# TIXhjq/ML_Function

Measured on AMD Instinct MI355X. Metric: samples/sec fwd+bwd xDeepFM-CIN B=4096,F=39,K=16, higher is better.
Workload: dtype f32

## Files before the change

ml_function_amd/csrc/cin.hip:

```cpp
#include "cin_layout.h"

namespace fil {

static const char* kFwdNames[kCinMaxL] = {"cin_fwd_l1", "cin_fwd_l2", "cin_fwd_l3", "cin_fwd_l4", "cin_fwd_l5", "cin_fwd_l6", "cin_fwd_l7", "cin_fwd_l8"};
static const char* kDwNames[kCinMaxL] = {"cin_bwd_dw_l1", "cin_bwd_dw_l2", "cin_bwd_dw_l3", "cin_bwd_dw_l4", "cin_bwd_dw_l5", "cin_bwd_dw_l6", "cin_bwd_dw_l7", "cin_bwd_dw_l8"};
static const char* kDzNames[kCinMaxL] = {"cin_bwd_dz_l1", "cin_bwd_dz_l2", "cin_bwd_dz_l3", "cin_bwd_dz_l4", "cin_bwd_dz_l5", "cin_bwd_dz_l6", "cin_bwd_dz_l7", "cin_bwd_dz_l8"};
static double gemm_flops(long M, int Hp, int F, int H) { return 2.0 * (double)M * Hp * F * H; }

static int launch_dw3(hipStream_t st, const DwPlan& p, const float* gT, int HS, const float* xT, const float* xpT, int xps, float* part,
                      long M, int F, int Hp, int H, int symD = 0, int xtra = 0) {
  const int items = p.blocks_x * p.splits * p.chunks;
  const dim3 grid((items + 7) / 8 * 8);
#define FIL_DW3(MBV, ONES) \
  hipLaunchKernelGGL((cin_dw3_kernel<MBV, ONES>), grid, dim3(kCinThreads), 0, st, gT, HS, xT, xpT, xps, part, (int)M, F, Hp, H, p.rows_per_split, \
                     p.blocks_x, p.chunks, items, symD, xtra)
  if (xT == nullptr) {
    if (p.MB == 2) FIL_DW3(2, true); else FIL_DW3(1, true);
  } else {
    if (p.MB == 2) FIL_DW3(2, false); else FIL_DW3(1, false);
  }
#undef FIL_DW3
  return p.splits;
}

// ... 461 lines not shown
struct CinBwd : CinCall {
  const float *pooled, *g;
  float* dx;
  float* const* dW;
  float* const* dbias;
  float *ddense_w, *ddense_b;
  void* const* events;
  CinBwdWs ws;
  const float* dPsrc;
  int nblk, ncol, ndc;
  int ready_slot[kCinMaxL + 1];
  int nready = 0;
  int cur = 0;
  int ltop;
  bool dx_started = false;
  bool have_gx0 = false;
  bool wz_prepacked = false;
  bool qm_joined = false;
};

static void cin_record_ready(const CinBwd& c, int slot) {
  if (c.events != nullptr && c.events[slot] != nullptr) (void)hipEventRecord((hipEvent_t)c.events[slot], c.st);
}
static void ready_next(CinBwd& c) { cin_record_ready(c, c.ready_slot[c.nready++]); }

static int cin_bwd_head(CinBwd& c) {
  const int B = c.s.B, LK = c.s.L * c.s.K;
  hipStream_t st = c.st;
  c.dPsrc = c.g;
  if (c.output_dim == 1 && c.p.qmerge) {
    c.dPsrc = c.ws.dP;
  } else if (c.output_dim == 1) {
    ProfScope ps("cin_head_bwd", st);
    hipLaunchKernelGGL(cin_head_bwd_kernel, dim3(c.nblk), dim3(256), 0, st, c.g, c.dense_w, c.pooled, c.ws.dP, c.ws.small, B, LK, kHeadChunk);
    if (!c.p.tail)
      hipLaunchKernelGGL(cin_reduce_kernel, dim3(cdiv(LK + 1, 64)), dim3(256), 0, st, c.ws.small, c.ddense_w, (long)(LK + 1), c.nblk, c.ddense_b, (long)LK);
    FIL_CIN_BWD_LAUNCHED();
    c.dPsrc = c.ws.dP;
  }
  if (!c.p.tail) ready_next(c);
  return FIL_OK;
}

static void cin_qtail_params_fill(const CinBwd& c) {
  const TailGeom& tg = c.p.tg;
  const CinBwdWs& ws = c.ws;
  const int F = c.s.F, p = tg.p, lL = c.s.L - 1, Hpp = tg.Hpp, Hq = tg.Hq;
  ProfScope ps("cin_tail_params", c.st);
  const size_t sh = cin_qtail_params_lds(F, Hq);
  allow_lds(cin_qtail_params_kernel, sh);
  float* dcfin = ws.dcpart + (size_t)c.ndc * kQtConst;
  hipLaunchKernelGGL(cin_qtail_params_kernel, dim3(2 * Hpp + 1), dim3(256), sh, c.st, c.W[p], c.sv.wsumL, ws.dT, ws.vlast, c.dW[p], ws.part, Hpp, F, Hq, ws.dcpart, c.ndc,
                     dcfin);
  hipLaunchKernelGGL(cin_qtail_fill_kernel, dim3(cdiv(Hq * F, kQtFillCols)), dim3(kQtFillThreads), 0, c.st, ws.part, Hpp, dcfin, c.bias[p], c.sv.wsumL, c.dW[lL], c.dbias[p],
                     c.dbias[lL], F, Hq, tg.HL);
}

static int cin_bwd_top_merged_q(CinBwd& c) {
  const CinShape& s = c.s;
  const TailGeom& tg = c.p.tg;
  const CinSaved& sv = c.sv;
  const CinBwdWs& ws = c.ws;
  const int F = s.F, K = s.K, L = s.L, JT = s.JT(), LK = s.L * s.K, *H = s.H;
  const long M = s.M();
  const bool qsplit = c.p.qsplit;
  const float* xT = c.xT;
  hipStream_t st = c.st;
  const int p = tg.p, lL = L - 1, Hpp = tg.Hpp, Hq = tg.Hq, HS0 = s.HS(0);
  FIL_CIN_CHECK_ARG(c.bias && c.W[0] && c.W[p] && c.W[lL] && c.bias[p] && c.dW[0] && c.dW[p] && c.dW[lL] && c.dbias[0] && c.dbias[p] && c.dbias[lL]);
  const float* xpT = sv.maps[p - 1];
  const int xps = s.xps(p);
  const float* dPp = c.dPsrc + (size_t)p * K;
  const float* dPL = c.dPsrc + (size_t)lL * K;
  const float* dPprev = c.dPsrc + (size_t)(p - 1) * K;
  const double algo_tail = gemm_flops(M, Hpp, F, Hq) + gemm_flops(M, Hq, F, tg.HL);
  const double algo1 = gemm_flops(M, F, F, H[0]);
  const int symD = F / 2 + 1, Cl = F * symD;
  const int JTs = cin_jt_sym(F);
  const int periods = cin_dz_periods(F, JTs), tiles0 = cin_slot_tiles(F, JTs);
  const bool ghat = cin_ghat_used(s, c.p, c.output_dim);
  const CinBwdWs::Scratch v = ws.scratch(s, true, ghat);
  const float* G = ghat ? sv.R : ws.G[c.cur];
  const float* gsc = ghat ? c.g : nullptr;
  {
    ProfScope ps("cin_tail_a", st, (double)M * (2 * F + 3) * sizeof(float));
    const size_t sh = (size_t)256 * (F + 3 + (c.output_dim == 1 ? L : 0) + (ghat ? 1 : 0)) * sizeof(float);
    allow_lds(cin_qtail_xe_kernel<3>, sh);
    allow_lds(cin_qtail_xe_kernel<1>, sh);
    const int np = (int)std::min<long>(((long)tiles0 * 32 * HS0 + 255) / 256, 1024);
    const int nq2 = qsplit ? 2 * std::min(cdiv(tiles0 * 512, 256), 256) : 0;
    if (c.p.qnp == 1)
      hipLaunchKernelGGL(cin_qtail_xe_kernel<1>, dim3(c.ndc + np + nq2), dim3(kXeThreads), sh, st, xT, dPL, dPp, LK, K, v.xr, ws.dcpart, (int)M, F,
                         c.ndc, c.output_dim == 1 ? c.g : nullptr, c.dense_w, c.pooled, ws.dP, ws.hpart, LK, lL, p, c.W[0], ws.Wz, H[0], JTs, HS0, tiles0, np, sv.T,
                         Hpp, ws.Wzb1, ws.Wzb2, ghat ? 1 : 0);
    else
      hipLaunchKernelGGL(cin_qtail_xe_kernel<3>, dim3(c.ndc + np + nq2), dim3(kXeThreads), sh, st, xT, dPL, dPp, LK, K, v.xr, ws.dcpart, (int)M, F,
                         c.ndc, c.output_dim == 1 ? c.g : nullptr, c.dense_w, c.pooled, ws.dP, ws.hpart, LK, lL, p, c.W[0], ws.Wz, H[0], JTs, HS0, tiles0, np, sv.T,
                         Hpp, ws.Wzb1, ws.Wzb2, ghat ? 1 : 0);
  }
  FIL_CIN_BWD_LAUNCHED();
  {
    ProfScope ps("cin_last_bwd", st, 6.0 * (double)M * Hpp * F);
    if (ghat)
      cin_launch_last_bwd2(st, JT, xT, xpT, xps, sv.wsumP, sv.wsnP, dPp, LK, nullptr, nullptr, HS0, ws.dxT, (int)M, F, K, Hpp);
    else
      cin_launch_last_bwd2(st, JT, xT, xpT, xps, sv.wsumP, sv.wsnP, dPp, LK, dPprev, ws.G[c.cur], HS0, ws.dxT, (int)M, F, K, Hpp, sv.R, HS0, dPL, ws.small);
  }
  FIL_CIN_BWD_LAUNCHED();
  int dw_parts = 0;
  {
    ProfScope ps("cin_bwd_dw_q", st, algo1 + algo_tail, gemm_flops(M, 1, Cl, H[0]) + gemm_flops(M, 1, Cl, Hpp));
    if (qsplit) {
      const DwqbPlan bp = cin_dwqb_plan(M, Cl + F, cu_count());
      cin_launch_dwq_b(st, c.p.qnp, bp, G, xpT, HS0, v.xr, v.XS, ws.part, (int)M, F, symD);
      dw_parts = bp.splits;
    } else {
      const bool f4 = knobs().dwfold4 != 0;
      const int Cw = Cl + F + (ghat ? 1 : 0);
      const DwqPlan dp = f4 ? cin_dwq_plan4(M, Cw, cu_count()) : cin_dwq_plan(M, Cw, cu_count());
#define FIL_DWQ(FOLDV, GHV) \
  hipLaunchKernelGGL((cin_dwq_kernel<kDwqDepth, FOLDV, GHV>), dim3((dp.wgs + 7) / 8 * 8), dim3(kDwqThreads), 0, st, G, xpT, HS0, v.xr, v.XS, ws.part, (int)M, F, \
                     symD, dp.rows_per_split, dp.splits, dp.ncol_full, dp.rem, dp.wgs_full, dp.wgs)
      if (ghat) {
        if (f4) FIL_DWQ(4, true); else FIL_DWQ(2, true);
      } else {
        if (f4) FIL_DWQ(4, false); else FIL_DWQ(2, false);
      }
#undef FIL_DWQ
      dw_parts = dp.pairs;
    }
  }
  FIL_CIN_BWD_LAUNCHED();
  {
    ProfScope ps("cin_reduce_dw", st);
    const int nb1 = ghat ? 0 : cdiv(H[0], 64);
    const int nh = c.output_dim == 1 ? cdiv(LK + 1, 64) : 0;
    if (ghat)
      hipLaunchKernelGGL(cin_reduce_expand_q_kernel<true>, dim3((Cl + F + 1 + 3) / 4 + nh), dim3(256), 0, st, ws.part, dw_parts, F, symD, H[0], Hpp, c.dW[0], ws.dT,
                         ws.vlast, ws.small, c.ncol, c.dbias[0], nb1, ws.hpart, c.ndc, LK, c.ddense_w, c.ddense_b);
    else
      hipLaunchKernelGGL(cin_reduce_expand_q_kernel<false>, dim3((Cl + F + 3) / 4 + nb1 + nh), dim3(256), 0, st, ws.part, dw_parts, F, symD, H[0], Hpp, c.dW[0], ws.dT,
                         ws.vlast, ws.small, c.ncol, c.dbias[0], nb1, ws.hpart, c.ndc, LK, c.ddense_w, c.ddense_b);
  }
  FIL_CIN_BWD_LAUNCHED();
  ready_next(c);
  ready_next(c);
  cin_qtail_params_fill(c);
  FIL_CIN_BWD_LAUNCHED();
  ready_next(c);
  ready_next(c);
  const int NHMAX = HS0 / 2;
  if (NHMAX == 64 && knobs().dz2 != 0) {
    ProfScope ps("cin_bwd_dz_q", st, algo1 + algo_tail, gemm_flops(M, 1, Cl, H[0]) + gemm_flops(M, 1, Cl, Hpp));
    bool split_done = false;
    if (qsplit) {
      split_done = cin_launch_dz2_b(st, c.p.qnp, JTs, G, xpT, HS0, dPL, LK, K, ws.Wzb1, ws.Wzb2, xT, ws.dxT, 1, (int)M, F, H[0], Hpp, periods, c.dx, sv.cvec);
    }
    if (!split_done &&
        !cin_launch_dz2(st, JTs, G, xpT, HS0, dPL, LK, K, ws.Wz, sv.WzT, xT, ws.dxT, 1, (int)M, F, H[0], Hpp, periods, c.dx, sv.cvec, gsc))
      return fail(FIL_ERR_UNSUPPORTED, "fil_cin_bwd: no two-pass data-gradient kernel for JT=%d (F=%d)", JTs, F);
    c.qm_joined = true;
  } else {
    const DzsShape z = dzs_launch_shape(c.p.tune, M, JTs, NHMAX);
    {
      ProfScope ps("cin_bwd_dz_tail", st, algo_tail, gemm_flops(M, 1, Cl, Hpp));
      cin_launch_dz3_sym(st, z.MBs, JTs, NHMAX, z.grid, xpT, HS0, sv.WzT, xT, v.gxR, v.dxR, 0, (int)M, F, Hpp, periods, z.ks);
    }
    FIL_CIN_BWD_LAUNCHED();
    {
      ProfScope ps("cin_bwd_dz_l1", st, algo1, gemm_flops(M, 1, Cl, H[0]));
      cin_launch_dz3_sym(st, z.MBs, JTs, NHMAX, z.grid, G, HS0, ws.Wz, xT, ws.gx0T, ws.dxT, 1, (int)M, F, H[0], periods, z.ks);
    }
    c.have_gx0 = true;
  }
  FIL_CIN_BWD_LAUNCHED();
  c.dx_started = true;
  c.ltop = -1;
  return FIL_OK;
}

static int cin_bwd_top_qtail(CinBwd& c) {
  const CinShape& s = c.s;
  const TailGeom& tg = c.p.tg;
  const CinSaved& sv = c.sv;
// ... 334 lines not shown
```

ml_function_amd/csrc/cin_layout.h:

```cpp
#pragma once
#include "cin_kernels.h"
#include "cin_tail.h"
#include "cin_launch.h"
#include "cin_qtail.h"
#include "cin_qsplit.h"
#include "cin_qmerge.h"

#include <stdlib.h>

namespace fil {

struct CinShape {
  int B, F, K, L;
  int H[kCinMaxL];
  int Hp(int l) const { return l == 0 ? F : H[l - 1]; }
  int HS(int l) const { return 128 * cdiv(H[l], 128); }
  int xps(int l) const { return l == 0 ? F : HS(l - 1); }
  long M() const { return (long)B * K; }
  int JT() const { return cin_jt_of(F); }
  int HSmax() const {
    int h = 0;
    for (int l = 0; l < L; ++l) h = std::max(h, HS(l));
    return h;
  }
};

static int check_shape(const char* fn, int B, int F, int K, int L, const int* H, CinShape& s) {
  if (B < 0 || F < 1 || K < 1 || L < 1 || H == nullptr) return fail(FIL_ERR_ARG, "%s: bad shape B=%d F=%d K=%d L=%d", fn, B, F, K, L);
  if (L > kCinMaxL) return fail(FIL_ERR_UNSUPPORTED, "%s: L=%d > %d", fn, L, kCinMaxL);
  if (F > kCinMaxFields) return fail(FIL_ERR_UNSUPPORTED, "%s: F=%d > %d fields", fn, F, kCinMaxFields);
  if ((long)B * K > (1L << 28)) return fail(FIL_ERR_UNSUPPORTED, "%s: B*K = %ld rows > 2^28 (row-split byte offsets of the dW kernel are 32-bit)", fn, (long)B * K);
  s.B = B; s.F = F; s.K = K; s.L = L;
  for (int l = 0; l < L; ++l) {
    if (H[l] < 1) return fail(FIL_ERR_ARG, "%s: H[%d]=%d", fn, l, H[l]);
    if (H[l] > kCinMaxH) return fail(FIL_ERR_UNSUPPORTED, "%s: H[%d]=%d > %d feature maps", fn, l, H[l], kCinMaxH);
    s.H[l] = H[l];
  }
  return FIL_OK;
}

static int chunks_of(int H) { return cdiv(H, 128); }
static int env_int(const char* name, int dflt) {
  const char* v = getenv(name);
  return v != nullptr && *v != 0 ? atoi(v) : dflt;
}
struct Knobs {
  int mb, sym, dw_mb, dw_splits, dz_mb, tail_splits, tail_settle, tail_dz_mode, ksplit, dzs_mb, qtail, qmerge, dz2, fwdq, headfold, packfold, dwfold4, ghat;
};
static const Knobs& knobs() {
  static const Knobs k = {env_int("FIL_CIN_MB", 0), env_int("FIL_CIN_SYM", 1), env_int("FIL_CIN_DW_MB", 1), env_int("FIL_CIN_DW_SPLITS", 0),
                          env_int("FIL_CIN_DZ_MB", 1), env_int("FIL_CIN_TAIL_SPLITS", 0), env_int("FIL_CIN_TAIL_SETTLE", 0), env_int("FIL_CIN_TAIL_DZ_MODE", 0), env_int("FIL_CIN_KSPLIT", -1), env_int("FIL_CIN_DZS_MB", 0), env_int("FIL_CIN_QTAIL", 1), env_int("FIL_CIN_QMERGE", 1), env_int("FIL_CIN_DZ2", 1), env_int("FIL_CIN_FWDQ", 1), env_int("FIL_CIN_HEADFOLD", 1), env_int("FIL_CIN_PACKFOLD", 1), env_int("FIL_CIN_DWFOLD4", 1), env_int("FIL_CIN_GHAT", 1)};
  return k;
}
struct CinTune {
  int mb_forced;
  bool sym, no_ksplit;
  CinTune() : CinTune(0) {}
  explicit CinTune(int mode)
      : mb_forced((mode & FIL_CIN_MB2) ? 2 : knobs().mb), sym(knobs().sym != 0 && !(mode & FIL_CIN_NOSYM)), no_ksplit((mode & FIL_CIN_NOKSPLIT) != 0) {}
  int mb_rows(long M) const {
    if (mb_forced == 1 || mb_forced == 2) return mb_forced;
    return cdiv((int)std::min<long>(M, 1L << 30), 64) >= 768 ? 2 : 1;
  }
  int ksplit(long M) const {
    if (knobs().ksplit == 0 || no_ksplit) return 1;
    if (mb_rows(M) != 1) return 1;
    if (knobs().ksplit == 4) return 4;
    return cdiv((int)std::min<long>(M, 1L << 30), 32) <= 512 ? 4 : 1;
  }
};

struct DwPlan {
  int MB, blocks_x, splits, rows_per_split, chunks;
};
static int cu_count() {
  static const int n = [] {
    int dev = 0, v = 0;
    if (hipGetDevice(&dev) != hipSuccess || hipDeviceGetAttribute(&v, hipDeviceAttributeMultiprocessorCount, dev) != hipSuccess || v <= 0) v = 256;
    return v;
  }();
  return n;
}

static DwPlan dw_plan(long M, int C, int H) {
  DwPlan p;
  p.chunks = chunks_of(H);
  p.MB = knobs().dw_mb == 2 ? 2 : 1;
  const int waves_c = cdiv(C, 32 * p.MB);
  p.blocks_x = cdiv(waves_c, 4);
  const long tiles = (long)p.blocks_x * p.chunks;
  const long ncu = cu_count();
  const long unit = 2 * kDwDepth;
  auto rows_of = [&](int splits) { return std::max<long>(unit, ((M + splits - 1) / splits + unit - 1) / unit * unit); };
  int best = knobs().dw_splits;
  if (best <= 0) {
    static const double t_of[4] = {0.0, 1.05e-4, 1.39e-4, 1.96e-4};
    double best_ms = -1.0;
    for (int sp = (int)std::max<long>(1, (M + (1L << 20) - 1) >> 20); sp <= 256; ++sp) {
      const long rps = rows_of(sp);
      const long real = (M + rps - 1) / rps;
      if (real != sp && sp > 1) continue;
      long wgs = tiles * real;
      double per_row = 0.0;
      while (wgs > 0) {
        const long round = std::min(wgs, 3 * ncu);
        per_row += t_of[std::min<long>(3, (round + ncu - 1) / ncu)];
        wgs -= round;
      }
      const double ms = (double)rps * per_row * p.MB + (double)real * C * H * 4.0 / 6e9;
      if (best_ms < 0 || ms < best_ms) best = sp, best_ms = ms;
      if (rps == unit) break;
    }
  }
  best = std::min(std::max(best, 1), 256);
  const long rps = rows_of(best);
  p.rows_per_split = (int)rps;
  p.splits = (int)std::max<long>(1, (M + rps - 1) / rps);
  return p;
}

struct TailGeom {
  bool on = false;
  int p = 0;
  int NCB = 0, JP = 0, JT4 = 0, NQ = 0, JHp = 0;
  int Hpp = 0, Hq = 0, HL = 0, Cp = 0, C1 = 0;
  int periods = 0, tiles = 0;
  size_t uf_floats = 0, uz_floats = 0;
};
static TailGeom tail_geom(const CinShape& s) {
  TailGeom g;
  if (s.L < 3 || !cin_tail_supported(s.F)) return g;
  g.on = true;
  g.p = s.L - 2;
  g.NCB = cin_tail_ncb(s.F);
// ... 192 lines not shown
```

ml_function_amd/csrc/cin_qmerge.h:

```cpp
#pragma once
#include "cin_kernels.h"
#include "cin_launch.h"
#include "cin_qtail.h"

namespace fil {

constexpr int kDwqDepth = 6;
constexpr int kDwqThreads = 512;
struct DwqPlan {
  int tiles, ncol_full, rem, splits, pairs, rows_per_split, wgs_full, wgs;
};
inline int cin_dwq_rem_wgs(int rem, int pairs) { return rem == 0 ? 0 : (rem == 1 ? (pairs + 3) / 4 : (rem == 2 ? (pairs + 1) / 2 : pairs)); }
inline DwqPlan cin_dwq_plan(long M, int C, int cus) {
  DwqPlan p;
  p.tiles = (C + 31) / 32;
  p.ncol_full = p.tiles / 4;
  p.rem = p.tiles % 4;
  const long unit = 2 * kDwqDepth;
  const long slots = cus;
  int best = 1;
  for (int s = 1; s <= 512; ++s) {
    if ((long)p.ncol_full * s + cin_dwq_rem_wgs(p.rem, s) > slots) break;
    best = s;
  }
// ... 191 lines not shown
  }
  float* pout = part + (long)pair * C * 256;
#pragma unroll
  for (int reg = 0; reg < 16; ++reg) {
    const int cr = c0 + mfma32_row(reg, half);
    if (cr < C) {
      float* dst = pout + (long)cr * 256 + 4 * r;
      if (cr < Cp || (GHAT && cr == C - 1)) *reinterpret_cast<float4*>(dst) = make_float4(acc[0][reg], acc[1][reg], acc[2][reg], acc[3][reg]);
      *reinterpret_cast<float4*>(dst + 128) = make_float4(acc[4][reg], acc[5][reg], acc[6][reg], acc[7][reg]);
    }
  }
}

template <bool GHAT = false>
static __global__ __launch_bounds__(256) void cin_reduce_expand_q_kernel(const float* __restrict__ part, int parts, int F, int D, int H1, int H2,
                                                                          float* __restrict__ dW1, float* __restrict__ dT, float* __restrict__ vT,
                                                                          const float* __restrict__ bpart, int nbp, float* __restrict__ dbias1,
                                                                          int nb1, const float* __restrict__ hpart, int nhp, int LK,
                                                                          float* __restrict__ ddw, float* __restrict__ ddb) {
  const int Cp = F * D, C = Cp + F + (GHAT ? 1 : 0);
  const int nbw = (C + 3) / 4;
  if ((int)blockIdx.x >= nbw + nb1) {
    cin_reduce_body(hpart, ddw, (long)LK + 1, nhp, ddb, (long)LK, (int)blockIdx.x - nbw - nb1);
    return;
  }
  if ((int)blockIdx.x >= nbw) {
    cin_reduce_body(bpart, dbias1, (long)H1, nbp, nullptr, 0, (int)blockIdx.x - nbw);
    return;
  }
  const int lane = threadIdx.x & 63, wave = threadIdx.x >> 6;
  const int c = blockIdx.x * 4 + wave;
  if (c >= C) return;
  const long ps = (long)C * 256;
  const float* p0 = part + (long)c * 256 + 4 * lane;
  f32x4 t[8];
#pragma unroll
  for (int u = 0; u < 8; ++u) t[u] = f32x4{0.f, 0.f, 0.f, 0.f};
  int p = 0;
  for (; p + 7 < parts; p += 8) {
#pragma unroll
    for (int u = 0; u < 8; ++u) t[u] += *reinterpret_cast<const f32x4*>(p0 + (long)(p + u) * ps);
  }
  for (; p < parts; ++p) t[0] += *reinterpret_cast<const f32x4*>(p0 + (long)p * ps);
  const f32x4 v = ((t[0] + t[1]) + (t[2] + t[3])) + ((t[4] + t[5]) + (t[6] + t[7]));
  const int col = 4 * lane, n0 = col & 127;
  const bool second = col >= 128;
  const int H = second ? H2 : H1;
  if (GHAT && c >= Cp + F) {
    if (!second) {
#pragma unroll
      for (int e = 0; e < 4; ++e)
        if (n0 + e < H1) dbias1[n0 + e] = v[e];
    }
    return;
  }
  if (c >= Cp) {
    if (second) {
#pragma unroll
      for (int e = 0; e < 4; ++e)
        if (n0 + e < H2) vT[(long)(c - Cp) * H2 + n0 + e] = v[e];
    }
    return;
  }
  const int h = c / D, d = c - h * D;
  const int f = (h + d) % F;
  float* dst = second ? dT : dW1;
  const bool twin = d != 0 && 2 * d != F;
  float* r0 = dst + ((long)h * F + f) * H + n0;
  float* r1 = dst + ((long)f * F + h) * H + n0;
  if ((H & 3) == 0 && n0 + 3 < H) {
    *reinterpret_cast<f32x4*>(r0) = v;
    if (twin) *reinterpret_cast<f32x4*>(r1) = v;
  } else {
#pragma unroll
    for (int e = 0; e < 4; ++e)
      if (n0 + e < H) {
        r0[e] = v[e];
        if (twin) r1[e] = v[e];
      }
  }
}

constexpr int kXeThreads = 1024;
template <int NP = 3>
static __global__ __launch_bounds__(kXeThreads) void cin_qtail_xe_kernel(const float* __restrict__ xT, const float* __restrict__ dPL,
                                                                  const float* __restrict__ dPp, int ldp, int K, float* __restrict__ xe,
                                                                  float* __restrict__ dcpart, int M, int F, int nscale,
                                                                  const float* __restrict__ g, const float* __restrict__ dense_w,
                                                                  const float* __restrict__ pooled, float* __restrict__ dP, float* __restrict__ hpart,
                                                                  int LK, int lL, int lp, const float* __restrict__ W0, float* __restrict__ Wz,
                                                                  int H0, int JTs, int HS0, int tiles0, int npz = -1,
                                                                  const float* __restrict__ Tq = nullptr, int HT = 0, u32x4* __restrict__ Wzb1 = nullptr,
                                                                  u32x4* __restrict__ Wzb2 = nullptr, int gcol = 0) {
  extern __shared__ __attribute__((aligned(16))) float smem[];
  if ((int)blockIdx.x >= nscale) {
    if (threadIdx.x >= 256) return;
    if (npz < 0) npz = gridDim.x - nscale;
    const int b = blockIdx.x - nscale;
    if (b < npz) cin_pack_wz_sym_body(W0, Wz, F, H0, JTs, HS0, tiles0, b, npz);
    else {
      const int nq = ((int)gridDim.x - nscale - npz) >> 1, q = b - npz;
      if (q < nq) cin_qs_pack_wz_body<NP>(W0, H0, Wzb1, tiles0, F, JTs, q, nq);
      else if (q < 2 * nq) cin_qs_pack_wz_body<NP>(Tq, HT, Wzb2, tiles0, F, JTs, q - nq, nq);
    }
    return;
  }
  const int nl = g != nullptr ? LK / K : 0;
  const int hl = nl + 1, XE = F + 3 + gcol;
  const int tid = threadIdx.x;
  const long m0 = (long)blockIdx.x * 256;
  const int nrows = (int)min((long)256, (long)M - m0);
  float* xs = smem;
  float* dls = xs + 256 * F;
  float* dps = dls + 256;
  float* hd = dps + 256;
  float* gs = hd + 256 * hl;
  {
    const float* src = xT + m0 * F;
    const int n = nrows * F;
    if ((reinterpret_cast<uintptr_t>(xT) & 15) == 0) {
      const int n4 = n >> 2;
      for (int i0 = tid; i0 < n4; i0 += 4 * kXeThreads) {
        float4 v[4];
#pragma unroll
        for (int u = 0; u < 4; ++u) v[u] = i0 + u * kXeThreads < n4 ? reinterpret_cast<const float4*>(src)[i0 + u * kXeThreads] : make_float4(0.f, 0.f, 0.f, 0.f);
#pragma unroll
        for (int u = 0; u < 4; ++u)
          if (i0 + u * kXeThreads < n4) reinterpret_cast<float4*>(xs)[i0 + u * kXeThreads] = v[u];
      }
      for (int i = 4 * n4 + tid; i < n; i += kXeThreads) xs[i] = src[i];
    } else {
      for (int i = tid; i < n; i += kXeThreads) xs[i] = src[i];
    }
    for (int i = n + tid; i < 256 * F; i += kXeThreads) xs[i] = 0.f;
  }
  if (tid < 256) {
    const long m = m0 + tid;
    float dl = 0.f, dp = 0.f, gr = 0.f;
    if (m < M) {
      const long b = m / K;
      const int k = (int)(m - b * K);
      if (g != nullptr) {
        const float gb = g[b];
        gr = gb;
        for (int l = 0; l < nl; ++l) {
          const float d = gb * dense_w[l * K + k];
          dP[b * LK + l * K + k] = d;
          hd[tid * hl + l] = gb * pooled[b * LK + l * K + k];
        }
        hd[tid * hl + nl] = k == 0 ? gb : 0.f;
        dl = gb * dense_w[lL * K + k];
        dp = gb * dense_w[lp * K + k];
      } else {
        dl = dPL[b * ldp + k];
        dp = dPp[b * ldp + k];
      }
    } else if (g != nullptr) {
      for (int l = 0; l <= nl; ++l) hd[tid * hl + l] = 0.f;
    }
    dls[tid] = dl;
    dps[tid] = dp;
    if (gcol) gs[tid] = gr;
  }
  __syncthreads();
  __shared__ float cs[4][64];
  if (tid < kXeThreads - 256) {
    constexpr int NT = kXeThreads - 256;
    float* dst = xe + m0 * XE;
    const int n4 = nrows * XE >> 2;
    const float rxe = 1.f / (float)XE;
    for (int i4 = tid; i4 < n4; i4 += NT) {
      int rr = (int)(((float)(4 * i4) + 0.5f) * rxe);
      int c = 4 * i4 - rr * XE;
      float e[4];
#pragma unroll
      for (int u = 0; u < 4; ++u) {
        e[u] = c < F ? xs[rr * F + c] : c == F ? 1.f : c == F + 1 ? dls[rr] : c == F + 2 ? dps[rr] : gs[rr];
        if (++c == XE) {
          c = 0;
          ++rr;
        }
      }
      reinterpret_cast<float4*>(dst)[i4] = make_float4(e[0], e[1], e[2], e[3]);
    }
    for (int i = 4 * n4 + tid; i < nrows * XE; i += NT) {
      const int rr = i / XE, c = i - rr * XE;
      dst[i] = c < F ? xs[rr * F + c] : c == F ? 1.f : c == F + 1 ? dls[rr] : c == F + 2 ? dps[rr] : gs[rr];
    }
  } else {
    const int t2 = tid - (kXeThreads - 256);
    {
      const int f = t2 & 63, q = t2 >> 6;
      float t0 = 0.f, t1 = 0.f;
      if (f < F) {
        for (int rr = 64 * q; rr < 64 * q + 64; rr += 2) {
          t0 += xs[rr * F + f] * dls[rr];
          t1 += xs[(rr + 1) * F + f] * dls[rr + 1];
        }
      } else if (f < F + 2) {
        const float* dv = f == F ? dls : dps;
        for (int rr = 64 * q; rr < 64 * q + 64; rr += 2) {
          t0 += dv[rr];
          t1 += dv[rr + 1];
        }
      }
      cs[q][f] = t0 + t1;
    }
    if (g != nullptr) {
      const int k0 = (int)(m0 % K);
      for (int j = t2; j <= LK; j += 256) {
        float t = 0.f;
        if (j < LK) {
          const int l = j / K, k = j - l * K;
          for (int rr = (k - k0 + K) % K; rr < 256; rr += K) t += hd[rr * hl + l];
        } else {
          for (int rr = (K - k0) % K; rr < 256; rr += K) t += hd[rr * hl + nl];
        }
        hpart[(long)blockIdx.x * (LK + 1) + j] = t;
      }
    }
  }
  __syncthreads();
  if (tid < F + 2) dcpart[(long)blockIdx.x * kQtConst + tid] = (cs[0][tid] + cs[1][tid]) + (cs[2][tid] + cs[3][tid]);
}

constexpr int kDz2FieldStride = 128 * 2;
inline int cin_dz2_rows(int F, int JT) {
  const int hpp = cin_dz_h_per_period(JT);
  return std::max(cin_dz_sym_rows(F, JT), (F + hpp - 1) / hpp * hpp);
}

__device__ __forceinline__ void cin_dz2_finish(const float* smem, int wave, int lane, int wrow0, int M, int F, int K, const float* __restrict__ dsc, int ldp,
                                               float* __restrict__ dxT, int accumulate, float* __restrict__ dx, const float* __restrict__ cvec) {
  constexpr int FS = kDz2FieldStride;
  const float* img = smem + wave * 32 * 2 + 1;
  const int nrow = min(32, M - wrow0);
  if (dx != nullptr) {
    const int rr = lane & 31;
    const int mm = wrow0 + rr;
    const bool ok = rr < nrow;
    const long mc = ok ? mm : M - 1;
    const long bb = mc / K;
    const int kk = (int)(mc - bb * K);
    const float sc = dsc[bb * ldp + kk];
    float* dxb = dx + (bb * F) * K + kk;
    const float* add = dxT + mc * F;
    for (int f0 = lane >> 5; f0 < F; f0 += 16) {
      float a8[8];
#pragma unroll
      for (int u = 0; u < 8; ++u) a8[u] = accumulate ? add[min(f0 + 2 * u, F - 1)] : 0.f;
#pragma unroll
      for (int u = 0; u < 8; ++u) {
        const int f = f0 + 2 * u;
        if (f < F) {
          const float v = a8[u] + img[f * FS + rr * 2] + sc * cvec[f];
          if (ok) dxb[(long)f * K] = v;
        }
      }
    }
    return;
  }
  float* dst = dxT + (long)wrow0 * F;
  for (int idx = lane; idx < nrow * F; idx += 64) {
    const int rr = idx / F, f = idx - rr * F;
    const float v = img[f * FS + rr * 2];
    dst[idx] = accumulate ? dst[idx] + v : v;
  }
}

template <int JT, int G>
__global__ __launch_bounds__(256, 2) void cin_dz2_kernel(const float* __restrict__ g1T, const float* __restrict__ g2T, int HS,
                                                         const float* __restrict__ dsc, int ldp, int K, const float* __restrict__ Wz1,
                                                         const float* __restrict__ Wz2, const float* __restrict__ xT, float* __restrict__ dxT,
                                                         int accumulate, int M, int F, int H1, int H2, int periods, int FR,
                                                         float* __restrict__ dx, const float* __restrict__ cvec,
                                                         const float* __restrict__ gsc = nullptr) {
  extern __shared__ __attribute__((aligned(16))) float smem[];
  constexpr int P = JT / gcd_c(16, JT);
  constexpr int HPP = 16 * P / JT;
  constexpr int NQ = 16;
  constexpr int FS = kDz2FieldStride;
  const int tid = threadIdx.x, lane = tid & 63, wave = tid >> 6;
  const int r = lane & 31, half = lane >> 5;
  const int wrow0 = (blockIdx.x * 4 + wave) * 32;
  if (wrow0 >= M) return;
  float* lrow = smem + (wave * 32 + r) * 2;
  const int m = wrow0 + r;
  const bool vq = m < M;
  const long mq = vq ? m : M - 1;
  f32x4s gq[16];
  {
    const f32x4s* grow4 = reinterpret_cast<const f32x4s*>(g1T + mq * HS + half * 64);
#pragma unroll
    for (int s4 = 0; s4 < 16; ++s4) gq[s4] = grow4[s4];
  }
  for (int f0 = half; f0 < FR; f0 += 16) {
    float xt[8];
#pragma unroll
    for (int u = 0; u < 8; ++u) xt[u] = xT[mq * F + min(f0 + 2 * u, F - 1)];
#pragma unroll
    for (int u = 0; u < 8; ++u) {
      const int f = f0 + 2 * u;
      if (f < FR) {
        const int keep = (vq && f < F) ? -1 : 0;
        *reinterpret_cast<float2*>(lrow + f * FS) = make_float2(__builtin_bit_cast(float, __builtin_bit_cast(int, xt[u]) & keep), 0.f);
      }
// ... 380 lines not shown
```

Before: 5.848 million.

## Fold last-layer shortcut dx backward into the qtail_xe kernel launch

When the ghat path is active, the separate cin_last_bwd launch is dropped. Its shortcut dx computation (xp times wsum via MFMA, scaled by g*dense_w) now runs as extra workgroups inside the cin_qtail_xe kernel, with several block-interleaving orders for mixing the shortcut and tail work. This removes one kernel launch and lets the two independent pieces of work overlap on the GPU. In exchange the fused kernel takes a larger LDS allocation, always uses the NP=3 variant, and changes launch bounds, which may hurt the occupancy of the original tail blocks.

```diff
diff --git a/ml_function_amd/csrc/cin.hip b/ml_function_amd/csrc/cin.hip
--- a/ml_function_amd/csrc/cin.hip
+++ b/ml_function_amd/csrc/cin.hip
@@ -567,24 +567,38 @@
   const CinBwdWs::Scratch v = ws.scratch(s, true, ghat);
   const float* G = ghat ? sv.R : ws.G[c.cur];
   const float* gsc = ghat ? c.g : nullptr;
-  {
-    ProfScope ps("cin_tail_a", st, (double)M * (2 * F + 3) * sizeof(float));
-    const size_t sh = (size_t)256 * (F + 3 + (c.output_dim == 1 ? L : 0) + (ghat ? 1 : 0)) * sizeof(float);
-    allow_lds(cin_qtail_xe_kernel<3>, sh);
-    allow_lds(cin_qtail_xe_kernel<1>, sh);
+  const bool scfold = ghat && knobs().shortcut_fold != 0;
+  {
+    ProfScope ps("cin_tail_a", st, (double)M * (2 * F + 3) * sizeof(float) + (scfold ? (double)M * (xps + F) * sizeof(float) : 0.0));
+    size_t sh = (size_t)256 * (F + 3 + (c.output_dim == 1 ? L : 0) + (ghat ? 1 : 0)) * sizeof(float);
     const int np = (int)std::min<long>(((long)tiles0 * 32 * HS0 + 255) / 256, 1024);
     const int nq2 = qsplit ? 2 * std::min(cdiv(tiles0 * 512, 256), 256) : 0;
-    if (c.p.qnp == 1)
-      hipLaunchKernelGGL(cin_qtail_xe_kernel<1>, dim3(c.ndc + np + nq2), dim3(kXeThreads), sh, st, xT, dPL, dPp, LK, K, v.xr, ws.dcpart, (int)M, F,
-                         c.ndc, c.output_dim == 1 ? c.g : nullptr, c.dense_w, c.pooled, ws.dP, ws.hpart, LK, lL, p, c.W[0], ws.Wz, H[0], JTs, HS0, tiles0, np, sv.T,
-                         Hpp, ws.Wzb1, ws.Wzb2, ghat ? 1 : 0);
-    else
-      hipLaunchKernelGGL(cin_qtail_xe_kernel<3>, dim3(c.ndc + np + nq2), dim3(kXeThreads), sh, st, xT, dPL, dPp, LK, K, v.xr, ws.dcpart, (int)M, F,
-                         c.ndc, c.output_dim == 1 ? c.g : nullptr, c.dense_w, c.pooled, ws.dP, ws.hpart, LK, lL, p, c.W[0], ws.Wz, H[0], JTs, HS0, tiles0, np, sv.T,
-                         Hpp, ws.Wzb1, ws.Wzb2, ghat ? 1 : 0);
-  }
-  FIL_CIN_BWD_LAUNCHED();
-  {
+    if (scfold) {
+      CinShortcutArgs sc;
+      sc.xpT = xpT, sc.wsum = sv.wsumP, sc.dxT = ws.dxT, sc.xps = xps, sc.Hp = Hpp;
+      sc.nwg = (int)((M + kScRows - 1) / kScRows);
+      const int kn = knobs().shortcut_fold;
+      sc.order = kn == 2 ? 0 : kn == 3 ? 1 : 2;
+      if (sc.order == 2 && c.ndc + np < sc.slots()) sc.order = 1;
+      sh = std::max(sh, cin_shortcut_lds(F, Hpp));
+      allow_lds(cin_qtail_xe_kernel<3, true, CinShortcutArgs>, sh);
+      hipLaunchKernelGGL((cin_qtail_xe_kernel<3, true, CinShortcutArgs>), dim3(c.ndc + np + sc.slots()), dim3(kXeThreads), sh, st, xT, dPL, dPp, LK, K, v.xr, ws.dcpart, (int)M, F, c.ndc, c.g,
+                         c.dense_w, c.pooled, ws.dP, ws.hpart, LK, lL, p, c.W[0], ws.Wz, H[0], JTs, HS0, tiles0, np, sv.T, Hpp, ws.Wzb1, ws.Wzb2, 1, sc);
+    } else {
+      allow_lds(cin_qtail_xe_kernel<3>, sh);
+      allow_lds(cin_qtail_xe_kernel<1>, sh);
+      if (c.p.qnp == 1)
+        hipLaunchKernelGGL(cin_qtail_xe_kernel<1>, dim3(c.ndc + np + nq2), dim3(kXeThreads), sh, st, xT, dPL, dPp, LK, K, v.xr, ws.dcpart, (int)M, F,
+                           c.ndc, c.output_dim == 1 ? c.g : nullptr, c.dense_w, c.pooled, ws.dP, ws.hpart, LK, lL, p, c.W[0], ws.Wz, H[0], JTs, HS0, tiles0, np, sv.T,
+                           Hpp, ws.Wzb1, ws.Wzb2, ghat ? 1 : 0);
+      else
+        hipLaunchKernelGGL(cin_qtail_xe_kernel<3>, dim3(c.ndc + np + nq2), dim3(kXeThreads), sh, st, xT, dPL, dPp, LK, K, v.xr, ws.dcpart, (int)M, F,
+                           c.ndc, c.output_dim == 1 ? c.g : nullptr, c.dense_w, c.pooled, ws.dP, ws.hpart, LK, lL, p, c.W[0], ws.Wz, H[0], JTs, HS0, tiles0, np, sv.T,
+                           Hpp, ws.Wzb1, ws.Wzb2, ghat ? 1 : 0);
+    }
+  }
+  FIL_CIN_BWD_LAUNCHED();
+  if (!scfold) {
     ProfScope ps("cin_last_bwd", st, 6.0 * (double)M * Hpp * F);
     if (ghat)
       cin_launch_last_bwd2(st, JT, xT, xpT, xps, sv.wsumP, sv.wsnP, dPp, LK, nullptr, nullptr, HS0, ws.dxT, (int)M, F, K, Hpp);
diff --git a/ml_function_amd/csrc/cin_layout.h b/ml_function_amd/csrc/cin_layout.h
--- a/ml_function_amd/csrc/cin_layout.h
+++ b/ml_function_amd/csrc/cin_layout.h
@@ -45,11 +45,11 @@
   return v != nullptr && *v != 0 ? atoi(v) : dflt;
 }
 struct Knobs {
-  int mb, sym, dw_mb, dw_splits, dz_mb, tail_splits, tail_settle, tail_dz_mode, ksplit, dzs_mb, qtail, qmerge, dz2, fwdq, headfold, packfold, dwfold4, ghat;
+  int mb, sym, dw_mb, dw_splits, dz_mb, tail_splits, tail_settle, tail_dz_mode, ksplit, dzs_mb, qtail, qmerge, dz2, fwdq, headfold, packfold, dwfold4, ghat, shortcut_fold;
 };
 static const Knobs& knobs() {
   static const Knobs k = {env_int("FIL_CIN_MB", 0), env_int("FIL_CIN_SYM", 1), env_int("FIL_CIN_DW_MB", 1), env_int("FIL_CIN_DW_SPLITS", 0),
-                          env_int("FIL_CIN_DZ_MB", 1), env_int("FIL_CIN_TAIL_SPLITS", 0), env_int("FIL_CIN_TAIL_SETTLE", 0), env_int("FIL_CIN_TAIL_DZ_MODE", 0), env_int("FIL_CIN_KSPLIT", -1), env_int("FIL_CIN_DZS_MB", 0), env_int("FIL_CIN_QTAIL", 1), env_int("FIL_CIN_QMERGE", 1), env_int("FIL_CIN_DZ2", 1), env_int("FIL_CIN_FWDQ", 1), env_int("FIL_CIN_HEADFOLD", 1), env_int("FIL_CIN_PACKFOLD", 1), env_int("FIL_CIN_DWFOLD4", 1), env_int("FIL_CIN_GHAT", 1)};
+                          env_int("FIL_CIN_DZ_MB", 1), env_int("FIL_CIN_TAIL_SPLITS", 0), env_int("FIL_CIN_TAIL_SETTLE", 0), env_int("FIL_CIN_TAIL_DZ_MODE", 0), env_int("FIL_CIN_KSPLIT", -1), env_int("FIL_CIN_DZS_MB", 0), env_int("FIL_CIN_QTAIL", 1), env_int("FIL_CIN_QMERGE", 1), env_int("FIL_CIN_DZ2", 1), env_int("FIL_CIN_FWDQ", 1), env_int("FIL_CIN_HEADFOLD", 1), env_int("FIL_CIN_PACKFOLD", 1), env_int("FIL_CIN_DWFOLD4", 1), env_int("FIL_CIN_GHAT", 1), env_int("FIL_CIN_SHORTCUT_FOLD", 1)};
   return k;
 }
 struct CinTune {
diff --git a/ml_function_amd/csrc/cin_qmerge.h b/ml_function_amd/csrc/cin_qmerge.h
--- a/ml_function_amd/csrc/cin_qmerge.h
+++ b/ml_function_amd/csrc/cin_qmerge.h
@@ -297,8 +297,106 @@
 }
 
 constexpr int kXeThreads = 1024;
-template <int NP = 3>
-static __global__ __launch_bounds__(kXeThreads) void cin_qtail_xe_kernel(const float* __restrict__ xT, const float* __restrict__ dPL,
+constexpr int kScCols = 16;
+constexpr int kScLd = kScCols + 2;
+constexpr int kScStage = 32 * kScLd;
+constexpr int kScWaves = 16, kScRows = 32 * kScWaves;
+inline size_t cin_shortcut_lds(int F, int Hp) { return ((size_t)((Hp * F + 3) & ~3) + (size_t)kScWaves * (kScStage + 32)) * sizeof(float); }
+struct CinShortcutArgs {
+  const float* xpT = nullptr;
+  const float* wsum = nullptr;
+  float* dxT = nullptr;
+  int xps = 0, Hp = 0;
+  int nwg = 0;
+  int order = 1;
+  __host__ __device__ int slots() const { return order == 2 ? (nwg + 7) & ~7 : nwg; }
+};
+__device__ __forceinline__ const CinShortcutArgs& cin_shortcut_args(const CinShortcutArgs& a) { return a; }
+template <bool TWO>
+__device__ __forceinline__ void cin_shortcut_dx_body(float* smem, int wg, const CinShortcutArgs& a, const float* __restrict__ g,
+                                                     const float* __restrict__ dense_w, int lp, int M, int F, int K) {
+  const float* __restrict__ xpT = a.xpT;
+  const int xps = a.xps, Hp = a.Hp;
+  const int tid = threadIdx.x, lane = tid & 63, wave = __builtin_amdgcn_readfirstlane(tid >> 6);
+  const int r = lane & 31, half = lane >> 5;
+  const int wrow0 = (wg * kScWaves + wave) * 32;
+  float* stg = smem + ((Hp * F + 3) & ~3) + wave * (kScStage + 32);
+  float* dps = stg + kScStage;
+  const int lrow = lane >> 2, c4 = lane & 3;
+  const bool live = wrow0 < M;
+  const __amdgpu_buffer_rsrc_t rx = make_rsrc_uniform(xpT + (live ? (long)wrow0 * xps : 0), live ? (long)min(32, M - wrow0) * xps * 4 : 0);
+  const int o0 = (lrow * xps + 4 * c4) * 4;
+  constexpr int kPast = 0x7ffffff0;
+  auto piece = [&](int c, int lower) {
+    const int vo = c * kScCols + 4 * c4 < xps ? o0 : kPast;
+    return __builtin_bit_cast(float4, __builtin_amdgcn_raw_buffer_load_b128(rx, vo, c * (kScCols * 4) + lower * (16 * xps * 4), 0));
+  };
+  float4 v0 = piece(0, 0), v1 = piece(0, 1);
+  for (int i = tid; i < Hp * F; i += kXeThreads) smem[i] = a.wsum[i];
+  if (live && half == 0) {
+    const long mq = min(wrow0 + r, M - 1);
+    const long b = mq / K;
+    const int k = (int)(mq - b * K);
+    dps[r] = g[b] * dense_w[lp * K + k];
+  }
+  __syncthreads();
+  if (!live) return;
+  f32x16 u0, u1;
+#pragma unroll
+  for (int i = 0; i < 16; ++i) u0[i] = u1[i] = 0.f;
+  const int quads = (Hp + 3) >> 2;
+  const int nch = (quads + 15) / 16 * (64 / kScCols);
+  constexpr int QC = kScCols / 4;
+  float* sdst = stg + lrow * kScLd + 4 * c4;
+  const float* xprow = stg + r * kScLd + 2 * half;
+  const float* wl0 = smem + 2 * half * F + min(r, F - 1);
+  const float* wl1 = smem + 2 * half * F + min(r + 32, F - 1);
+  const int qlast = (Hp - 1) & ~3;
+  auto andf = [](float w, int m) { return __builtin_bit_cast(float, __builtin_bit_cast(int, w) & m); };
+#pragma unroll 1
+  for (int c = 0; c < nch; ++c) {
+    __builtin_amdgcn_wave_barrier();
+    *reinterpret_cast<float2*>(sdst) = make_float2(v0.x, v0.y);
+    *reinterpret_cast<float2*>(sdst + 2) = make_float2(v0.z, v0.w);
+    *reinterpret_cast<float2*>(sdst + 16 * kScLd) = make_float2(v1.x, v1.y);
+    *reinterpret_cast<float2*>(sdst + 16 * kScLd + 2) = make_float2(v1.z, v1.w);
+    __builtin_amdgcn_wave_barrier();
+    if (c + 1 < nch) {
+      v0 = piece(c + 1, 0);
+      v1 = piece(c + 1, 1);
+    }
+    __builtin_amdgcn_sched_barrier(0);
+#pragma unroll
+    for (int i = 0; i < QC; ++i) {
+      float2 av = *reinterpret_cast<const float2*>(xprow + 4 * i);
+      const int qm = (c * QC + i - quads) >> 31;
+      av = make_float2(andf(av.x, qm), andf(av.y, qm));
+      const int hq = c * kScCols + 4 * i, h = hq + 2 * half;
+      const int ro = min(hq, qlast) * F;
+      const int k0 = (h - Hp) >> 31, k1 = (h + 1 - Hp) >> 31;
+      u0 = mfma32(av.x, andf(wl0[ro], k0), u0);
+      u0 = mfma32(av.y, andf(wl0[ro + F], k1), u0);
+      if constexpr (TWO) {
+        u1 = mfma32(av.x, andf(wl1[ro], k0), u1);
+        u1 = mfma32(av.y, andf(wl1[ro + F], k1), u1);
+      }
+    }
+  }
+  float* dxT = a.dxT;
+#pragma unroll
+  for (int reg = 0; reg < 16; ++reg) {
+    const int row = mfma32_row(reg, half);
+    const int m = wrow0 + row;
+    if (m < M) {
+      const float dpr = dps[row];
+      if (r < F) dxT[(long)m * F + r] = dpr * u0[reg];
+      if (TWO && r + 32 < F) dxT[(long)m * F + 32 + r] = dpr * u1[reg];
+    }
+  }
+}
+
+template <int NP = 3, bool SC = false, typename... ScArgs>
+static __global__ __launch_bounds__(kXeThreads, SC ? 8 : 1) void cin_qtail_xe_kernel(const float* __restrict__ xT, const float* __restrict__ dPL,
                                                                   const float* __restrict__ dPp, int ldp, int K, float* __restrict__ xe,
                                                                   float* __restrict__ dcpart, int M, int F, int nscale,
                                                                   const float* __restrict__ g, const float* __restrict__ dense_w,
@@ -306,15 +404,44 @@
                                                                   int LK, int lL, int lp, const float* __restrict__ W0, float* __restrict__ Wz,
                                                                   int H0, int JTs, int HS0, int tiles0, int npz = -1,
                                                                   const float* __restrict__ Tq = nullptr, int HT = 0, u32x4* __restrict__ Wzb1 = nullptr,
-                                                                  u32x4* __restrict__ Wzb2 = nullptr, int gcol = 0) {
+                                                                  u32x4* __restrict__ Wzb2 = nullptr, int gcol = 0, ScArgs... sca) {
   extern __shared__ __attribute__((aligned(16))) float smem[];
-  if ((int)blockIdx.x >= nscale) {
+  unsigned bid = blockIdx.x;
+  const auto grid = [&]() -> unsigned {
+    if constexpr (SC) return gridDim.x - (unsigned)cin_shortcut_args(sca...).slots();
+    else return gridDim.x;
+  };
+  if constexpr (SC) {
+    const CinShortcutArgs& sc = cin_shortcut_args(sca...);
+    int w = -1;
+    if (sc.order == 2) {
+      if ((int)bid < 2 * sc.slots()) {
+        const int idx = (int)(bid >> 4) * 8 + (int)(bid & 7);
+        if ((bid >> 3) & 1) bid = idx;
+        else if (idx < sc.nwg) w = idx;
+        else return;
+      } else {
+        bid -= sc.slots();
+      }
+    } else if (sc.order == 1) {
+      if ((int)bid < sc.nwg) w = bid;
+      else bid -= sc.nwg;
+    } else if (bid >= grid()) {
+      w = (int)(bid - grid());
+    }
+    if (w >= 0) {
+      if (F > 32) cin_shortcut_dx_body<true>(smem, w, sc, g, dense_w, lp, M, F, K);
+      else cin_shortcut_dx_body<false>(smem, w, sc, g, dense_w, lp, M, F, K);
+      return;
+    }
+  }
+  if ((int)bid >= nscale) {
     if (threadIdx.x >= 256) return;
-    if (npz < 0) npz = gridDim.x - nscale;
-    const int b = blockIdx.x - nscale;
+    if (npz < 0) npz = grid() - nscale;
+    const int b = bid - nscale;
     if (b < npz) cin_pack_wz_sym_body(W0, Wz, F, H0, JTs, HS0, tiles0, b, npz);
     else {
-      const int nq = ((int)gridDim.x - nscale - npz) >> 1, q = b - npz;
+      const int nq = ((int)grid() - nscale - npz) >> 1, q = b - npz;
       if (q < nq) cin_qs_pack_wz_body<NP>(W0, H0, Wzb1, tiles0, F, JTs, q, nq);
       else if (q < 2 * nq) cin_qs_pack_wz_body<NP>(Tq, HT, Wzb2, tiles0, F, JTs, q - nq, nq);
     }
@@ -323,7 +450,7 @@
   const int nl = g != nullptr ? LK / K : 0;
   const int hl = nl + 1, XE = F + 3 + gcol;
   const int tid = threadIdx.x;
-  const long m0 = (long)blockIdx.x * 256;
+  const long m0 = (long)bid * 256;
   const int nrows = (int)min((long)256, (long)M - m0);
   float* xs = smem;
   float* dls = xs + 256 * F;
@@ -431,12 +558,12 @@
         } else {
           for (int rr = (K - k0) % K; rr < 256; rr += K) t += hd[rr * hl + nl];
         }
-        hpart[(long)blockIdx.x * (LK + 1) + j] = t;
+        hpart[(long)bid * (LK + 1) + j] = t;
       }
     }
   }
   __syncthreads();
-  if (tid < F + 2) dcpart[(long)blockIdx.x * kQtConst + tid] = (cs[0][tid] + cs[1][tid]) + (cs[2][tid] + cs[3][tid]);
+  if (tid < F + 2) dcpart[(long)bid * kQtConst + tid] = (cs[0][tid] + cs[1][tid]) + (cs[2][tid] + cs[3][tid]);
 }
 
 constexpr int kDz2FieldStride = 128 * 2;
```

Result: no change. 5.872 million (median of 4 runs) (+0.4%).
